# InternetMaximalism/plonky2_bn254

Hardware: AMD Instinct MI355X
Metric: G1 scalar-mul STARK proofs/sec (256-bit scalars) (higher is better)
Workload: dtype u64 (Goldilocks p = 2^64-2^32+1; BN254 Fq as 10x26-bit Montgomery limbs); 1 GPU; configs[1]: batch of 1024 G1 scalar-muls on 1 GPU per step = 8 proofs x 128 instances, 2^16 rows, W=781, standard_fast_config; instances_per_proof=128, steps_in_flight=4, parallelism=1 GPU, no collective

## Files before the change

plonky2_bn254_amd/csrc/quotient_common.h:

```cpp
#pragma once
#include "gl_dev.h"
#include "aux.h"

struct Acc {
  u64 lo, hi;
  u32 ov;
};
__device__ __forceinline__ void acc_init(Acc& a) {
  a.lo = 0;
  a.hi = 0;
  a.ov = 0;
}
__device__ __forceinline__ void acc_mad(Acc& a, u64 x, u64 w) {
  const unsigned __int128 pr = (unsigned __int128)x * w;
  u64 pl = (u64)pr, ph = (u64)(pr >> 64);
  a.lo += pl;
  u64 c = a.lo < pl ? 1 : 0;
  u64 h = a.hi + ph;
  u32 o = h < ph ? 1 : 0;
  h += c;
  o += h < c ? 1 : 0;
  a.hi = h;
  a.ov += o;
}
__device__ __forceinline__ u64 acc_red(const Acc& a) {
  return gl_sub(gl_reduce128(a.lo, a.hi), ((u64)a.ov) << 32);
}
struct Acc2 {
  Acc a0, a1;
};
__device__ __forceinline__ void acc2_init(Acc2& a) {
  acc_init(a.a0);
  acc_init(a.a1);
}
__device__ __forceinline__ void acc2_mad(Acc2& a, u64 x, u64 w0, u64 w1) {
  acc_mad(a.a0, x, w0);
  acc_mad(a.a1, x, w1);
}

static constexpr u32 M22 = (1u << 22) - 1;
struct W3 {
  u32 w0, w1, w2;
};
GL_HD W3 w3_split(u64 w) {
  W3 r;
  r.w0 = (u32)w & M22;
  r.w1 = (u32)(w >> 22) & M22;
  r.w2 = (u32)(w >> 44);
  return r;
}
struct Acc3 {
  u64 c[5];
};
__device__ __forceinline__ void acc3_init(Acc3& a) {
#pragma unroll
  for (int k = 0; k < 5; k++) a.c[k] = 0;
}
__device__ __forceinline__ void acc3_mad(Acc3& a, u32 v0, u32 v1, u32 v2, u32 w0, u32 w1, u32 w2) {
  a.c[0] += (u64)v0 * w0;
  a.c[1] += (u64)v0 * w1;
  a.c[1] += (u64)v1 * w0;
  a.c[2] += (u64)v0 * w2;
  a.c[2] += (u64)v1 * w1;
  a.c[2] += (u64)v2 * w0;
  a.c[3] += (u64)v1 * w2;
  a.c[3] += (u64)v2 * w1;
  a.c[4] += (u64)v2 * w2;
}
__device__ __forceinline__ u64 acc3_red(const Acc3& a) {
  unsigned __int128 t = (unsigned __int128)a.c[0] + ((unsigned __int128)a.c[1] << 22) + ((unsigned __int128)a.c[2] << 44);
  u64 r = gl_reduce128((u64)t, (u64)(t >> 64));
  r = gl_add(r, gl_mul_2exp<66>(gl_reduce128(a.c[3], 0)));
  r = gl_add(r, gl_mul_2exp<88>(gl_reduce128(a.c[4], 0)));
  return r;
}

struct AccW {
  Acc3 a0, a1;
};
__device__ __forceinline__ void accw_init(AccW& a) {
  acc3_init(a.a0);
  acc3_init(a.a1);
}
__device__ __forceinline__ void accw_mad(AccW& a, u64 x, const u32* __restrict__ w) {
  const u32 v0 = (u32)x & M22, v1 = (u32)(x >> 22) & M22, v2 = (u32)(x >> 44);
  acc3_mad(a.a0, v0, v1, v2, w[0], w[1], w[2]);
  acc3_mad(a.a1, v0, v1, v2, w[4], w[5], w[6]);
}
GL_HD void w3_store(u64* dst , u64 wa, u64 wb) {
  const W3 a = w3_split(wa), b = w3_split(wb);
  dst[0] = (u64)a.w0 | ((u64)a.w1 << 32);
  dst[1] = (u64)a.w2;
  dst[2] = (u64)b.w0 | ((u64)b.w1 << 32);
  dst[3] = (u64)b.w2;
}

struct QPointTables {
  const u64* x;
  const u64* lfirst;
  const u64* llast;
};

__device__ __forceinline__ size_t next_position(size_t j, unsigned log_n) {
  const size_t N = (size_t)1 << log_n;
  size_t h = j >> log_n;
  u32 k = bitrev32((u32)(j & (N - 1)), log_n);
  k = (k + 1) & (u32)(N - 1);
  return (h << log_n) | bitrev32(k, log_n);
}

__device__ __forceinline__ void lookup_and_ctl_constraints(const StarkShape& sh, const u64* __restrict__ tl,
                                                           const u64* __restrict__ al, size_t M2, size_t j, size_t jn,
                                                           const u32* __restrict__ W3 , int e0,
                                                           const u64 betas[2], const u64 gammas[2], u64 lfirst, u64 llast,
                                                           u64 z_last, u64& tot0, u64& tot1) {
  const int m = sh.n_helpers(), n_rc = sh.n_rc();
  int e = e0;
  AccW acc;
  accw_init(acc);
  const u64 table = tl[(size_t)sh.table_col * M2 + j], freq = tl[(size_t)sh.freq_col * M2 + j];
  u64 hs[2] = {0, 0};
#pragma unroll 4
  for (int k = 0; k < m; k++) {
    u64 f0 = tl[(size_t)(sh.rc_begin + 2 * k) * M2 + j];
    bool two = (2 * k + 1) < n_rc;
    u64 f1 = two ? tl[(size_t)(sh.rc_begin + 2 * k + 1) * M2 + j] : 0;
#pragma unroll
    for (int ch = 0; ch < 2; ch++) {
      u64 h = al[(size_t)(ch * (m + 1) + k) * M2 + j];
      u64 g0 = gl_add(f0, betas[ch]);
      u64 c;
      if (two) {
        u64 g1 = gl_add(f1, betas[ch]);
        c = gl_sub(gl_sub(gl_mul(gl_mul(g1, g0), h), g1), g0);
      } else {
        c = gl_sub(gl_mul(g0, h), 1);
      }
      int ee = e0 + ch * (m + 2) + k;
      accw_mad(acc, c, W3 + 8 * (ee));
      hs[ch] = gl_add(hs[ch], h);
    }
  }
#pragma unroll
  for (int ch = 0; ch < 2; ch++) {
    u64 z = al[(size_t)(ch * (m + 1) + m) * M2 + j], nz = al[(size_t)(ch * (m + 1) + m) * M2 + jn];
    u64 twc = gl_add(table, betas[ch]);
    u64 y = gl_sub(gl_mul(hs[ch], twc), freq);
    int ee = e0 + ch * (m + 2) + m;
    accw_mad(acc, gl_mul(z, lfirst), W3 + 8 * (ee));
    accw_mad(acc, gl_sub(gl_mul(gl_sub(nz, z), twc), y), W3 + 8 * (ee + 1));
  }
  e = e0 + 2 * (m + 2);
  for (int ctl = 0; ctl < sh.n_ctl; ctl++) {
    u64 a0 = 0, a1 = 0;
    for (int mm = sh.ctl.ncols[ctl] - 1; mm >= 0; mm--) {
      int start = sh.ctl.col_start[ctl][mm], nb = sh.ctl.col_bits[ctl][mm];
      u64 v = 0;
      for (int b = nb - 1; b >= 0; b--) v = gl_add(gl_dbl(v), tl[(size_t)(start + b) * M2 + j]);
      a0 = gl_add(gl_mul(a0, betas[0]), v);
      a1 = gl_add(gl_mul(a1, betas[1]), v);
    }
    u64 comb[2] = {gl_add(a0, gammas[0]), gl_add(a1, gammas[1])};
    u64 f0 = tl[(size_t)sh.ctl.filter_col[ctl] * M2 + j];
#pragma unroll
    for (int ch = 0; ch < 2; ch++) {
      int zc = 2 * (m + 1) + ctl * 2 + ch;
      u64 lz = al[(size_t)zc * M2 + j], nz = al[(size_t)zc * M2 + jn];
      u64 c_last = gl_mul(gl_sub(gl_mul(comb[ch], lz), f0), llast);
      u64 c_tr = gl_mul(gl_sub(gl_mul(comb[ch], gl_sub(lz, nz)), f0), z_last);
      accw_mad(acc, c_last, W3 + 8 * (e));
      accw_mad(acc, c_tr, W3 + 8 * (e + 1));
      e += 2;
    }
  }
  tot0 = gl_add(tot0, acc3_red(acc.a0));
  tot1 = gl_add(tot1, acc3_red(acc.a1));
}
```

plonky2_bn254_amd/csrc/quotient_g1.hip:

```cpp
#include "quotient_sched.h"
#include "trace_g1.h"
#include "quotient.h"

static constexpr int G1_K_AIR = 1111;
static constexpr int G1_MZ_E0[5] = {0, 50, 83, 132, 165};

__global__ __launch_bounds__(256, 2) void k_quotient_g1_sched(QArgs A) {
  const size_t j = (size_t)blockIdx.x * blockDim.x + threadIdx.x;
  if (j >= A.count) return;
  schedule_part<G1L, false>(A, j, q_next(A, j), 198, 5);
}

template <int part>
__global__ __launch_bounds__(256, 2) void k_quotient_g1_add(QArgs A) {
  const size_t M2 = A.stride;
  const size_t j = (size_t)blockIdx.x * blockDim.x + threadIdx.x;
  if (j >= A.count) return;
  const u64* __restrict__ tl = A.tl;
  const u64* __restrict__ W0 = A.W;
  const u64* __restrict__ W1 = A.W + A.K;
  const u32* __restrict__ W3 = (const u32*)(A.W + 2 * (size_t)A.K);
  u64 tot0 = 0, tot1 = 0;
  int e = 0;
  const int AUX = G1_COL_AUX;
  const u64 filter = TL(G1_COL_FILTER);
  const u64 is_x_eq_filter = TL(AUX + G1_AUX_IS_X_EQ_FILTER);
  u64 ax[16], lam[16], t16[16], u16[16];
  ld16(tl, M2, j, G1_COL_A, ax);
  if constexpr (part == 0) {
    const u64 is_x_eq = TL(AUX + G1_AUX_IS_X_EQ);
    ld16(tl, M2, j, G1_COL_B, u16);
#pragma unroll
    for (int i = 0; i < 16; i++) u16[i] = gl_sub(u16[i], ax[i]);
    ld16(tl, M2, j, AUX + G1_AUX_IS_X_EQ_AUX, t16);
    const u64 c0 = gl_sub(is_x_eq, 1);
    mz_block<true>(tl, M2, j, AUX + G1_AUX_IS_X_EQ_AUX + 16, A, G1_MZ_E0[0], 0,
             filter, [&](int i) __attribute__((always_inline)) { u64 v = conv16<true>(u16, t16, i); return i == 0 ? gl_add(v, c0) : v; }, tot0, tot1);
    e = 33;
    AccW g;
    accw_init(g);
#pragma unroll
    for (int i = 0; i < 16; i++) accw_mad(g, u16[i], W3 + 8 * (e + i));
    e += 16;
    u64 f = gl_mul(filter, is_x_eq);
    tot0 = gl_add(tot0, gl_mul(f, acc3_red(g.a0)));
    tot1 = gl_add(tot1, gl_mul(f, acc3_red(g.a1)));
    EMIT(gl_sub(gl_mul(filter, is_x_eq), is_x_eq_filter));
  } else if constexpr (part == 1) {
    ld16(tl, M2, j, AUX + G1_AUX_LAMBDA, lam);
    ld16(tl, M2, j, G1_COL_B, u16);
#pragma unroll
    for (int i = 0; i < 16; i++) u16[i] = gl_sub(u16[i], ax[i]);
    ld16(tl, M2, j, G1_COL_B + 16, t16);
    ld16(tl, M2, j, G1_COL_A + 16, ax);
    mz_block<true>(tl, M2, j, AUX + G1_AUX_LAMBDA_AUX, A, G1_MZ_E0[1], 1,
             gl_sub(filter, is_x_eq_filter),
             [&](int i) __attribute__((always_inline)) {
               u64 v = conv16<true>(lam, u16, i);
               return i < 16 ? gl_sub(v, gl_sub(t16[i < 16 ? i : 0], ax[i < 16 ? i : 0])) : v;
             },
             tot0, tot1);
  } else if constexpr (part == 2) {
    ld16(tl, M2, j, AUX + G1_AUX_LAMBDA, lam);
    ld16(tl, M2, j, G1_COL_A + 16, u16);
    mz_block<true>(tl, M2, j, AUX + G1_AUX_LAMBDA_AUX, A, G1_MZ_E0[2], 2,
             is_x_eq_filter,
             [&](int i) __attribute__((always_inline)) {
               u64 ly = conv16<true>(lam, u16, i), xx = conv16<true>(ax, ax, i);
               return gl_sub(gl_dbl(ly), gl_add(gl_dbl(xx), xx));
             },
             tot0, tot1);
    e = 116;
    ld16(tl, M2, j, G1_COL_B + 16, t16);
    AccW g;
    accw_init(g);
#pragma unroll
    for (int i = 0; i < 16; i++) accw_mad(g, gl_sub(u16[i], t16[i]), W3 + 8 * (e + i));
    tot0 = gl_add(tot0, gl_mul(is_x_eq_filter, acc3_red(g.a0)));
    tot1 = gl_add(tot1, gl_mul(is_x_eq_filter, acc3_red(g.a1)));
  } else if constexpr (part == 3) {
    ld16(tl, M2, j, AUX + G1_AUX_LAMBDA, lam);
    ld16(tl, M2, j, G1_COL_B, t16);
    ld16(tl, M2, j, G1_COL_C, u16);
    mz_block<true>(tl, M2, j, AUX + G1_AUX_X_AUX, A, G1_MZ_E0[3], 3, filter,
             [&](int i) __attribute__((always_inline)) {
               u64 v = conv16<true>(lam, lam, i);
               return i < 16 ? gl_sub(v, gl_add(gl_add(ax[i < 16 ? i : 0], t16[i < 16 ? i : 0]), u16[i < 16 ? i : 0])) : v;
             },
             tot0, tot1);
  } else {
    ld16(tl, M2, j, AUX + G1_AUX_LAMBDA, lam);
    ld16(tl, M2, j, G1_COL_C, u16);
#pragma unroll
    for (int i = 0; i < 16; i++) u16[i] = gl_sub(u16[i], ax[i]);
    ld16(tl, M2, j, G1_COL_C + 16, t16);
    ld16(tl, M2, j, G1_COL_A + 16, ax);
    mz_block<true>(tl, M2, j, AUX + G1_AUX_Y_AUX, A, G1_MZ_E0[4], 4, filter,
             [&](int i) __attribute__((always_inline)) {
               u64 v = conv16<true>(lam, u16, i);
               return i < 16 ? gl_add(v, gl_add(t16[i < 16 ? i : 0], ax[i < 16 ? i : 0])) : v;
             },
             tot0, tot1);
  }
  store_part(A, part, j, tot0, tot1);
}

__global__ __launch_bounds__(256) void k_quotient_finish(QArgs A, StarkShape sh) {
  const size_t j = (size_t)blockIdx.x * blockDim.x + threadIdx.x;
  if (j >= A.count) return;
  finish_point(A, sh, j);
}
void quotient_finish_launch(const QArgs& A, const StarkShape& sh, hipStream_t st) {
  k_quotient_finish<<<(unsigned)((A.count + 255) / 256), 256, 0, st>>>(A, sh);
}

__global__ void k_point_tables(u64* x, u64* lfirst, u64* llast, unsigned log_n, u64 w_n, u64 w_2n) {
  const size_t N = (size_t)1 << log_n;
  size_t j = (size_t)blockIdx.x * blockDim.x + threadIdx.x;
  if (j >= 2 * N) return;
  size_t h = j >> log_n;
  u32 k = bitrev32((u32)(j & (N - 1)), log_n);
  u64 shift = h ? gl_mul(GL_GEN, w_2n) : GL_GEN;
  u64 xv = gl_mul(shift, gl_pow(w_n, k));
  u64 gn = gl_pow(GL_GEN, N);
  u64 zh = gl_sub(h ? gl_neg(gn) : gn, 1);
  u64 ninv = gl_inv((u64)N % GL_P);
  u64 winv = gl_inv(w_n);
  x[j] = xv;
  lfirst[j] = gl_mul(gl_mul(zh, ninv), gl_inv(gl_sub(xv, 1)));
  llast[j] = gl_mul(gl_mul(gl_mul(zh, ninv), winv), gl_inv(gl_sub(xv, winv)));
}

__global__ void k_point_tables_window(u64* x, u64* lfirst, u64* llast, unsigned log_n, u32 h, size_t k0, size_t count, u64 w_n,
                                      u64 w_2n) {
  const size_t N = (size_t)1 << log_n;
  size_t j = (size_t)blockIdx.x * blockDim.x + threadIdx.x;
  if (j >= count) return;
  const u64 k = (k0 + j) & (N - 1);
  u64 shift = h ? gl_mul(GL_GEN, w_2n) : GL_GEN;
  u64 xv = gl_mul(shift, gl_pow(w_n, k));
  u64 gn = gl_pow(GL_GEN, N);
  u64 zh = gl_sub(h ? gl_neg(gn) : gn, 1);
  u64 ninv = gl_inv((u64)N % GL_P);
  u64 winv = gl_inv(w_n);
  x[j] = xv;
  lfirst[j] = gl_mul(gl_mul(zh, ninv), gl_inv(gl_sub(xv, 1)));
  llast[j] = gl_mul(gl_mul(gl_mul(zh, ninv), winv), gl_inv(gl_sub(xv, winv)));
}
void quotient_point_tables_window(u64* d_x, u64* d_lfirst, u64* d_llast, unsigned log_n, int h, size_t k0, size_t count, hipStream_t st) {
  k_point_tables_window<<<(unsigned)((count + 255) / 256), 256, 0, st>>>(d_x, d_lfirst, d_llast, log_n, (u32)h, k0, count,
                                                                       gl_root_of_unity(log_n), gl_root_of_unity(log_n + 1));
}
void quotient_window_args(QArgs& A, const u64* d_tw, const u64* d_aw, const QPointTables& pt, u64* d_part, size_t stride, size_t count,
                          size_t k0, int h) {
  A.tl = d_tw;
  A.al = d_aw;
  A.pt = pt;
  A.part = d_part;
  A.stride = stride;
  A.count = count;
  A.k0 = k0;
  A.natural = 1;
  A.hsel = (u32)h;
}

void quotient_point_tables(u64* d_x, u64* d_lfirst, u64* d_llast, unsigned log_n, hipStream_t st) {
  size_t M2 = (size_t)2 << log_n;
  k_point_tables<<<(unsigned)((M2 + 255) / 256), 256, 0, st>>>(d_x, d_lfirst, d_llast, log_n, gl_root_of_unity(log_n),
                                                             gl_root_of_unity(log_n + 1));
}

void quotient_host_tables(int K, const u64 alphas[2], const int* mz_e0, int n_blocks, std::vector<u64>& W, std::vector<u64>& mzt) {
  W.assign(QUOTIENT_W_WORDS(K), 0);
  for (int a = 0; a < 2; a++) {
    u64 v = 1;
    for (int e = K - 1; e >= 0; e--) {
      W[(size_t)a * K + e] = v;
      v = gl_mul(v, alphas[a]);
    }
  }
  static const u64 MOD[16] = {64839, 55420, 35862, 15392, 51853, 26737, 27281, 38785,
                              22621, 33153, 17846, 47184, 41001, 57649, 20082, 12388};
  const u64 B = 1ULL << 16, OFF = 1ULL << 29;
  mzt.assign(QUOTIENT_MZT_WORDS, 0);
  for (int blk = 0; blk < n_blocks; blk++)
    for (int a = 0; a < 2; a++) {
      const u64* w = &W[(size_t)a * K + mz_e0[blk] + 1];
      u64* T = &mzt[(size_t)(blk * 2 + a) * 80];
      for (int jj = 0; jj < 17; jj++) {
        u64 s = 0;
        for (int t = 0; t < 16; t++)
          if (jj + t < 32) s = gl_add(s, gl_mul(w[jj + t], MOD[t]));
        T[jj] = s;
      }
      u64 usum = 0;
      for (int d = 0; d < 31; d++) {
        u64 u = gl_sub(w[d + 1], gl_mul(B, w[d]));
        T[17 + d] = u;
        T[48 + d] = gl_mul(B, u);
        usum = gl_add(usum, u);
      }
      T[79] = gl_mul(OFF, usum);
    }
  for (int e = 0; e < K; e++) w3_store(&W[2 * (size_t)K + 4 * (size_t)e], W[e], W[(size_t)K + e]);
  for (int blk = 0; blk < n_blocks; blk++)
    for (int t = 0; t < 80; t++)
      w3_store(&mzt[QUOTIENT_MZT3_OFF + (size_t)(blk * 80 + t) * 4], mzt[(size_t)(blk * 2) * 80 + t], mzt[(size_t)(blk * 2 + 1) * 80 + t]);
}

void quotient_fill_args(QArgs& A, const StarkShape& sh, const u64* d_tl, const u64* d_al, const u64* d_W, const u64* d_mzt,
                        const QPointTables& pt, const u64 betas[2], const u64 gammas[2], unsigned log_n, u64* d_out,
                        u64* d_part) {
  A.tl = d_tl;
  A.al = d_al;
  A.W = d_W;
  A.mzt = d_mzt;
  A.pt = pt;
  for (int i = 0; i < 2; i++) {
    A.betas[i] = betas[i];
    A.gammas[i] = gammas[i];
  }
  const size_t N = (size_t)1 << log_n;
  u64 gn = gl_pow(GL_GEN, N);
  A.zh_inv[0] = gl_inv(gl_sub(gn, 1));
  A.zh_inv[1] = gl_inv(gl_sub(gl_neg(gn), 1));
  A.w_inv = gl_inv(gl_root_of_unity(log_n));
  A.out = d_out;
  A.part = d_part;
  A.n_parts = 0;
  A.log_n = log_n;
  A.K = sh.n_total_constraints();
  A.stride = A.count = 2 * N;
  A.k0 = 0;
  A.natural = 0;
  A.hsel = 0;
}

int g1_quotient_mz_blocks(const int** e0) {
  *e0 = G1_MZ_E0;
  return 5;
}
void g1_quotient_launch(const QArgs& A0, const StarkShape& sh, hipStream_t st) {
  QArgs A = A0;
  A.n_parts = 6;
  const unsigned g = (unsigned)((A.count + 255) / 256);
  k_quotient_g1_add<0><<<g, 256, 0, st>>>(A);
  k_quotient_g1_add<1><<<g, 256, 0, st>>>(A);
  k_quotient_g1_add<2><<<g, 256, 0, st>>>(A);
  k_quotient_g1_add<3><<<g, 256, 0, st>>>(A);
  k_quotient_g1_add<4><<<g, 256, 0, st>>>(A);
  k_quotient_g1_sched<<<g, 256, 0, st>>>(A);
  quotient_finish_launch(A, sh, st);
}

void quotient_g1_module_warm() {
  hipFuncAttributes a;
  (void)hipFuncGetAttributes(&a, reinterpret_cast<const void*>(&k_point_tables));
}
```

plonky2_bn254_amd/csrc/quotient_g2fq.hip:

```cpp
#include "quotient_sched.h"
#include "quotient.h"

static constexpr int G2_MZ_E0[10] = {1, 50, 100, 133, 166, 199, 264, 297, 330, 363};
static constexpr int FQ_MZ_E0[1] = {0};

__device__ __forceinline__ u64 econv_c0(const u64* x0, const u64* x1, const u64* y0, const u64* y1, int i) {
  return gl_sub(conv16(x0, y0, i), conv16(x1, y1, i));
}
__device__ __forceinline__ u64 econv_c1(const u64* x0, const u64* x1, const u64* y0, const u64* y1, int i) {
  return gl_add(conv16(x0, y1, i), conv16(x1, y0, i));
}

#define MZB(blk, auxcol, FILTER, FN, ...) \
  mz_block(tl, M2, j, (auxcol), A, G2_MZ_E0[blk], (blk), (FILTER), FN, tot0, tot1, ##__VA_ARGS__)

__global__ __launch_bounds__(256, 2) void k_quotient_g2_sched(QArgs A) {
  const size_t j = (size_t)blockIdx.x * blockDim.x + threadIdx.x;
  if (j >= A.count) return;
  schedule_part<G2L, false>(A, j, q_next(A, j), 396, 6);
}

template <int part>
__global__ __launch_bounds__(256, 2) void k_quotient_g2_add(QArgs A) {
  typedef G2L L;
  const size_t M2 = A.stride;
  const size_t j = (size_t)blockIdx.x * blockDim.x + threadIdx.x;
  if (j >= A.count) return;
  const u64* __restrict__ tl = A.tl;
  const u64* __restrict__ W0 = A.W;
  const u64* __restrict__ W1 = A.W + A.K;
  const u32* __restrict__ W3 = (const u32*)(A.W + 2 * (size_t)A.K);
  u64 tot0 = 0, tot1 = 0;
  int e = 0;
  const u64 filter = TL(L::FILTER);
  const int AUX = L::AUX;
  u64 is_x_eq_filter = 0;
  if constexpr (part == 1 || part == 2) is_x_eq_filter = TL(AUX + G2_AUX_IS_X_EQ_FILTER);
  auto seed_w = [&](Acc2& sd, int blk, int i, u64 v) { acc2_mad(sd, v, W0[G2_MZ_E0[blk] + 1 + i], W1[G2_MZ_E0[blk] + 1 + i]); };
  if constexpr (part == 0 || part == 5) {
    constexpr int h = part == 0 ? 0 : 1;
    u64 dx[16], t0[16];
    const u64 z = TL(AUX + (h ? G2_AUX_IS_C1_ZERO : G2_AUX_IS_C0_ZERO));
    if constexpr (h == 0) {
      EMIT(gl_mul(filter, gl_sub(gl_mul(z, TL(AUX + G2_AUX_IS_C1_ZERO)), TL(AUX + G2_AUX_IS_X_EQ))));
    }
#pragma unroll
    for (int i = 0; i < 16; i++) dx[i] = gl_sub(TL(L::B + 16 * h + i), TL(L::A + 16 * h + i));
    ld16(tl, M2, j, AUX + (h ? G2_AUX_C1_AUX : G2_AUX_C0_AUX), t0);
    const u64 c0 = gl_sub(z, 1);
    MZB(h, AUX + (h ? G2_AUX_C1_AUX : G2_AUX_C0_AUX) + 16, filter, [&](int i) __attribute__((always_inline)) { u64 v = conv16(dx, t0, i); return i == 0 ? gl_add(v, c0) : v; });
    e = h ? 83 : 34;
    AccW g;
    accw_init(g);
#pragma unroll
    for (int i = 0; i < 16; i++) accw_mad(g, dx[i], W3 + 8 * (e + i));
    const u64 f = gl_mul(filter, z);
    tot0 = gl_add(tot0, gl_mul(f, acc3_red(g.a0)));
    tot1 = gl_add(tot1, gl_mul(f, acc3_red(g.a1)));
    if constexpr (h == 1) {
      e = 99;
      EMIT(gl_sub(gl_mul(filter, TL(AUX + G2_AUX_IS_X_EQ)), TL(AUX + G2_AUX_IS_X_EQ_FILTER)));
    }
  } else {
    Acc2 sd0, sd1;
    acc2_init(sd0);
    acc2_init(sd1);
    u64 l0[16], l1[16], dx0[16], dx1[16];
    if constexpr (part == 1) {
#pragma unroll 4
      for (int i = 0; i < 16; i++) seed_w(sd0, 2, i, gl_sub(TL(L::A + 32 + i), TL(L::B + 32 + i)));
      ld16(tl, M2, j, AUX + G2_AUX_LAMBDA, l0);
      ld16(tl, M2, j, AUX + G2_AUX_LAMBDA + 16, l1);
#pragma unroll
      for (int i = 0; i < 16; i++) {
        dx0[i] = gl_sub(TL(L::B + i), TL(L::A + i));
        dx1[i] = gl_sub(TL(L::B + 16 + i), TL(L::A + 16 + i));
      }
      const u64 f_ne = gl_sub(filter, is_x_eq_filter);
      MZB(2, AUX + G2_AUX_LAMBDA_AUX, f_ne, [&](int i) __attribute__((always_inline)) { return econv_c0(l0, l1, dx0, dx1, i); }, &sd0);
#pragma unroll 4
      for (int i = 0; i < 16; i++) seed_w(sd1, 3, i, gl_sub(TL(L::A + 48 + i), TL(L::B + 48 + i)));
      MZB(3, AUX + G2_AUX_LAMBDA_AUX + 80, f_ne, [&](int i) __attribute__((always_inline)) { return econv_c1(l0, l1, dx0, dx1, i); }, &sd1);
    } else if constexpr (part == 2) {
      ld16(tl, M2, j, L::A, dx0);
      ld16(tl, M2, j, L::A + 16, dx1);
#pragma unroll
      for (int i = 0; i < 31; i++) {
        const u64 xx0 = econv_c0(dx0, dx1, dx0, dx1, i), xx1 = econv_c1(dx0, dx1, dx0, dx1, i);
        seed_w(sd0, 4, i, gl_neg(gl_add(gl_dbl(xx0), xx0)));
        seed_w(sd1, 5, i, gl_neg(gl_add(gl_dbl(xx1), xx1)));
      }
      ld16(tl, M2, j, AUX + G2_AUX_LAMBDA, l0);
      ld16(tl, M2, j, AUX + G2_AUX_LAMBDA + 16, l1);
      ld16(tl, M2, j, L::A + 32, dx0);
      ld16(tl, M2, j, L::A + 48, dx1);
      MZB(4, AUX + G2_AUX_LAMBDA_AUX, is_x_eq_filter, [&](int i) __attribute__((always_inline)) { return gl_dbl(econv_c0(l0, l1, dx0, dx1, i)); }, &sd0);
      MZB(5, AUX + G2_AUX_LAMBDA_AUX + 80, is_x_eq_filter, [&](int i) __attribute__((always_inline)) { return gl_dbl(econv_c1(l0, l1, dx0, dx1, i)); }, &sd1);
      e = 232;
      AccW g;
      accw_init(g);
#pragma unroll
      for (int i = 0; i < 16; i++) accw_mad(g, gl_sub(dx0[i], TL(L::B + 32 + i)), W3 + 8 * (e + i));
#pragma unroll
      for (int i = 0; i < 16; i++) accw_mad(g, gl_sub(dx1[i], TL(L::B + 48 + i)), W3 + 8 * (e + 16 + i));
      tot0 = gl_add(tot0, gl_mul(is_x_eq_filter, acc3_red(g.a0)));
      tot1 = gl_add(tot1, gl_mul(is_x_eq_filter, acc3_red(g.a1)));
    } else if constexpr (part == 3) {
#pragma unroll 4
      for (int i = 0; i < 16; i++) {
        seed_w(sd0, 6, i, gl_neg(gl_add(gl_add(TL(L::A + i), TL(L::B + i)), TL(L::C + i))));
        seed_w(sd1, 7, i, gl_neg(gl_add(gl_add(TL(L::A + 16 + i), TL(L::B + 16 + i)), TL(L::C + 16 + i))));
      }
      ld16(tl, M2, j, AUX + G2_AUX_LAMBDA, l0);
      ld16(tl, M2, j, AUX + G2_AUX_LAMBDA + 16, l1);
      MZB(6, AUX + G2_AUX_X_AUX, filter, [&](int i) __attribute__((always_inline)) { return econv_c0(l0, l1, l0, l1, i); }, &sd0);
      MZB(7, AUX + G2_AUX_X_AUX + 80, filter, [&](int i) __attribute__((always_inline)) { return econv_c1(l0, l1, l0, l1, i); }, &sd1);
    } else {
#pragma unroll 4
      for (int i = 0; i < 16; i++) seed_w(sd0, 8, i, gl_add(TL(L::C + 32 + i), TL(L::A + 32 + i)));
      ld16(tl, M2, j, AUX + G2_AUX_LAMBDA, l0);
      ld16(tl, M2, j, AUX + G2_AUX_LAMBDA + 16, l1);
#pragma unroll
      for (int i = 0; i < 16; i++) {
        dx0[i] = gl_sub(TL(L::C + i), TL(L::A + i));
        dx1[i] = gl_sub(TL(L::C + 16 + i), TL(L::A + 16 + i));
      }
      MZB(8, AUX + G2_AUX_Y_AUX, filter, [&](int i) __attribute__((always_inline)) { return econv_c0(l0, l1, dx0, dx1, i); }, &sd0);
#pragma unroll 4
      for (int i = 0; i < 16; i++) seed_w(sd1, 9, i, gl_add(TL(L::C + 48 + i), TL(L::A + 48 + i)));
      MZB(9, AUX + G2_AUX_Y_AUX + 80, filter, [&](int i) __attribute__((always_inline)) { return econv_c1(l0, l1, dx0, dx1, i); }, &sd1);
    }
  }
  store_part(A, part, j, tot0, tot1);
}

__global__ __launch_bounds__(256, 2) void k_quotient_fq_sched(QArgs A) {
  const size_t j = (size_t)blockIdx.x * blockDim.x + threadIdx.x;
  if (j >= A.count) return;
  schedule_part<FQL, true>(A, j, q_next(A, j), 33, 1);
}
__global__ __launch_bounds__(256) void k_quotient_fq_mul(QArgs A) {
  typedef FQL L;
  const size_t M2 = A.stride;
  const size_t j = (size_t)blockIdx.x * blockDim.x + threadIdx.x;
  if (j >= A.count) return;
  const u64* __restrict__ tl = A.tl;
  const u64* __restrict__ W0 = A.W;
  const u64* __restrict__ W1 = A.W + A.K;
  u64 tot0 = 0, tot1 = 0;
  const u64 filter = TL(L::FILTER);
  u64 a[16], b[16], c[16];
  ld16(tl, M2, j, L::A, a);
  ld16(tl, M2, j, L::B, b);
  ld16(tl, M2, j, L::C, c);
  mz_block(tl, M2, j, L::AUX, A, FQ_MZ_E0[0], 0, filter,
           [&](int i) __attribute__((always_inline)) {
             u64 v = conv16(a, b, i);
             return i < 16 ? gl_sub(v, c[i < 16 ? i : 0]) : v;
           },
           tot0, tot1);
  store_part(A, 0, j, tot0, tot1);
}

int g2_quotient_mz_blocks(const int** e0) {
  *e0 = G2_MZ_E0;
  return 10;
}
int fq_quotient_mz_blocks(const int** e0) {
  *e0 = FQ_MZ_E0;
  return 1;
}
void g2_quotient_launch(const QArgs& A0, const StarkShape& sh, hipStream_t st) {
  QArgs A = A0;
  A.n_parts = 7;
  const unsigned g = (unsigned)((A.count + 255) / 256);
  k_quotient_g2_add<0><<<g, 256, 0, st>>>(A);
  k_quotient_g2_add<5><<<g, 256, 0, st>>>(A);
  k_quotient_g2_add<1><<<g, 256, 0, st>>>(A);
  k_quotient_g2_add<2><<<g, 256, 0, st>>>(A);
  k_quotient_g2_add<3><<<g, 256, 0, st>>>(A);
  k_quotient_g2_add<4><<<g, 256, 0, st>>>(A);
  k_quotient_g2_sched<<<g, 256, 0, st>>>(A);
  quotient_finish_launch(A, sh, st);
}
void fq_quotient_launch(const QArgs& A0, const StarkShape& sh, hipStream_t st) {
  QArgs A = A0;
  A.n_parts = 2;
  const unsigned g = (unsigned)((A.count + 255) / 256);
  k_quotient_fq_mul<<<g, 256, 0, st>>>(A);
  k_quotient_fq_sched<<<g, 256, 0, st>>>(A);
  quotient_finish_launch(A, sh, st);
}

void quotient_g2fq_module_warm() {
  hipFuncAttributes a;
  (void)hipFuncGetAttributes(&a, reinterpret_cast<const void*>(&k_quotient_fq_sched));
}
```

plonky2_bn254_amd/csrc/quotient_sched.h:

```cpp
#pragma once
#include <vector>
#include "quotient_common.h"
#include "layout.h"

#ifndef MZ_CONSTS
#define MZ_CONSTS
static constexpr int QMZ_IQP = 0, QMZ_QUOT = 1, QMZ_LO = 18, QMZ_HI = 49;
#endif

struct QArgs {
  const u64* tl;
  const u64* al;
  const u64* W;
  const u64* mzt;
  QPointTables pt;
  u64 betas[2], gammas[2];
  u64 zh_inv[2];
  u64 w_inv;
  u64* out;
  u64* part;
  int n_parts;
  unsigned log_n;
  int K;
  size_t stride, count, k0;
  u32 natural, hsel;
};
static constexpr size_t QUOTIENT_MZT3_OFF = 10 * 2 * 80, QUOTIENT_MZT_WORDS = 10 * 2 * 80 + 10 * 80 * 4;
static inline size_t QUOTIENT_W_WORDS(int K) { return 6 * (size_t)K; }
__device__ __forceinline__ size_t q_next(const QArgs& A, size_t j) { return A.natural ? j + 1 : next_position(j, A.log_n); }

#define TL(c) tl[(size_t)(c)*M2 + j]
#define TN(c) tl[(size_t)(c)*M2 + jn]

__device__ __forceinline__ void ld16(const u64* __restrict__ tl, size_t M2, size_t j, int col, u64* v) {
#pragma unroll
  for (int i = 0; i < 16; i++) v[i] = tl[(size_t)(col + i) * M2 + j];
}
template <bool FULL = false>
__device__ __forceinline__ u64 conv16(const u64* A, const u64* B, int i) {
  Acc a;
  acc_init(a);
  if constexpr (FULL) {
#pragma clang loop unroll(full)
    for (int s = 0; s < 16; s++) {
      int t = i - s;
      if (t >= 0 && t < 16) acc_mad(a, A[s], B[t]);
    }
  } else {
#pragma unroll
    for (int s = 0; s < 16; s++) {
      int t = i - s;
      if (t >= 0 && t < 16) acc_mad(a, A[s], B[t]);
    }
  }
  return acc_red(a);
}

template <bool FULL = false, class InFn>
__device__ __forceinline__ void mz_block(const u64* __restrict__ tl, size_t M2, size_t j, int auxcol, const QArgs& A, int e0, int blk,
                                         u64 filter, InFn in, u64& tot0, u64& tot1, const Acc2* seed = nullptr) {
  const u64* __restrict__ w0 = A.W + e0;
  const u64* __restrict__ w1 = A.W + A.K + e0;
  const u64* __restrict__ T0 = A.mzt + (size_t)blk * 160;
  const u64* __restrict__ T1 = T0 + 80;
  const u32* __restrict__ w3 = (const u32*)(A.W + 2 * (size_t)A.K) + 8 * (size_t)e0;
  const u32* __restrict__ T3 = (const u32*)(A.mzt + QUOTIENT_MZT3_OFF) + 8 * (size_t)(blk * 80);
  u64 n0, n1;
  {
    Acc2 neg;
    if (seed) neg = *seed;
    else acc2_init(neg);
    if constexpr (FULL) {
#pragma clang loop unroll(full)
      for (int i = 0; i < 31; i++) acc2_mad(neg, in(i), w0[1 + i], w1[1 + i]);
    } else {
#pragma unroll
      for (int i = 0; i < 31; i++) {
        acc2_mad(neg, in(i), w0[1 + i], w1[1 + i]);
        __builtin_amdgcn_sched_barrier(0);
      }
    }
    n0 = acc_red(neg.a0);
    n1 = acc_red(neg.a1);
  }
  __builtin_amdgcn_sched_barrier(0);
  const u64 iqp = TL(auxcol + QMZ_IQP);
  const u64 qsign = gl_sub(gl_dbl(iqp), 1);
  u64 s0, s1;
  {
    AccW q;
    accw_init(q);
#pragma unroll 1
    for (int jj = 0; jj < 17; jj++) accw_mad(q, TL(auxcol + QMZ_QUOT + jj), T3 + 8 * jj);
    s0 = gl_mul(qsign, acc3_red(q.a0));
    s1 = gl_mul(qsign, acc3_red(q.a1));
  }
  __builtin_amdgcn_sched_barrier(0);
  {
    AccW pos;
    accw_init(pos);
    accw_mad(pos, gl_sub(gl_mul(iqp, iqp), iqp), w3);
#pragma unroll 1
    for (int d = 0; d < 31; d++) {
      accw_mad(pos, TL(auxcol + QMZ_LO + d), T3 + 8 * (17 + d));
      accw_mad(pos, TL(auxcol + QMZ_HI + d), T3 + 8 * (48 + d));
    }
    s0 = gl_add(s0, acc3_red(pos.a0));
    s1 = gl_add(s1, acc3_red(pos.a1));
  }
  s0 = gl_sub(gl_sub(s0, T0[79]), n0);
  s1 = gl_sub(gl_sub(s1, T1[79]), n1);
  tot0 = gl_add(tot0, gl_mul(filter, s0));
  tot1 = gl_add(tot1, gl_mul(filter, s1));
  asm volatile("" : "+v"(tot0), "+v"(tot1));
}

#define EQ_GROUP(filter, n, AEXPR, BEXPR)                         \
  {                                                               \
    static_assert((n) % 16 == 0, "EQ_GROUP: n % 16");             \
    AccW g_;                                                      \
    accw_init(g_);                                                \
    constexpr int CH_ = 16;                                       \
    _Pragma("unroll 1") for (int i0_ = 0; i0_ < (n); i0_ += CH_) { \
      u64 d_[CH_];                                                \
      _Pragma("unroll") for (int k_ = 0; k_ < CH_; k_++) {        \
        const int i = i0_ + k_;                                   \
        d_[k_] = gl_sub((AEXPR), (BEXPR));                        \
      }                                                           \
      _Pragma("unroll") for (int k_ = 0; k_ < CH_; k_++) accw_mad(g_, d_[k_], W3 + 8 * (e + i0_ + k_)); \
    }                                                             \
    e += (n);                                                     \
    u64 f_ = (filter);                                            \
    tot0 = gl_add(tot0, gl_mul(f_, acc3_red(g_.a0)));             \
    tot1 = gl_add(tot1, gl_mul(f_, acc3_red(g_.a1)));             \
    asm volatile("" : "+v"(tot0), "+v"(tot1));  \
  }
#define EMIT(c)                                  \
  {                                              \
    u64 c_ = (c);                                \
    tot0 = gl_add(tot0, gl_mul(c_, W0[e]));      \
    tot1 = gl_add(tot1, gl_mul(c_, W1[e]));      \
    e += 1;                                      \
  }


__device__ __forceinline__ void store_part(const QArgs& A, int part, size_t j, u64 tot0, u64 tot1) {
  const size_t M2 = A.stride;
  A.part[((size_t)part * 2 + 0) * M2 + j] = tot0;
  A.part[((size_t)part * 2 + 1) * M2 + j] = tot1;
}

template <class L, bool FIRST_A_IS_ONE>
__device__ __forceinline__ void schedule_part(const QArgs& A, size_t j, size_t jn, int e, int part) {
  u64 tot0 = 0, tot1 = 0;
  const size_t M2 = A.stride;
  const u64* __restrict__ tl = A.tl;
  const u64* __restrict__ W0 = A.W;
  const u64* __restrict__ W1 = A.W + A.K;
  const u32* __restrict__ W3 = (const u32*)(A.W + 2 * (size_t)A.K);
  const u64 filter = TL(L::FILTER);
  const u64 is_first = TL(L::FLAGS + 0), is_last = TL(L::FLAGS + 1);
  const u64 n_filter = TN(L::FILTER), n_is_last = TN(L::FLAGS + 1);
  const u64 is_not_last_round = gl_sub(filter, is_last);
  const u64 is_next_not_last_round = gl_sub(n_filter, n_is_last);
  const u64 is_adding = TL(L::IS_ADDING), idnl = TL(L::IDNL);
  const u64 n_is_adding = TN(L::IS_ADDING), n_idnl = TN(L::IDNL);
  const u64 bit0 = TL(L::BITS), n_bit0 = TN(L::BITS);

  EMIT(gl_mul(is_first, gl_sub(is_adding, 1)));
  EQ_GROUP(is_first, L::PL, TL(L::DOUBLE + i), TL(L::B + i));
  EQ_GROUP(gl_mul(bit0, is_first), L::PL, TL(L::SUM + i), TL(L::C + i));
  EQ_GROUP(gl_mul(gl_sub(1, bit0), is_first), L::PL, TL(L::SUM + i), TL(L::A + i));
  if (FIRST_A_IS_ONE) {
    EQ_GROUP(is_first, L::PL, TL(L::A + i), (u64)(i == 0 ? 1 : 0));
  }
  EQ_GROUP(idnl, L::PL, TN(L::A + i), TL(L::SUM + i));
  EQ_GROUP(idnl, L::PL, TN(L::B + i), TL(L::DOUBLE + i));
  EQ_GROUP(gl_mul(n_bit0, idnl), L::PL, TN(L::SUM + i), TN(L::C + i));
  EQ_GROUP(gl_mul(gl_sub(1, n_bit0), idnl), L::PL, TN(L::SUM + i), TN(L::A + i));
  EQ_GROUP(idnl, L::PL, TN(L::DOUBLE + i), TL(L::DOUBLE + i));
  EMIT(gl_mul(idnl, gl_sub(n_is_adding, 1)));
  EMIT(gl_mul(idnl, n_idnl));
  EQ_GROUP(idnl, 256, TN(L::BITS + i), TL(L::BITS + ((i + 1) & 255)));
  EQ_GROUP(is_adding, L::PL, TN(L::A + i), TL(L::DOUBLE + i));
  EQ_GROUP(is_adding, L::PL, TN(L::B + i), TL(L::DOUBLE + i));
  EQ_GROUP(is_adding, L::PL, TN(L::SUM + i), TL(L::SUM + i));
  EQ_GROUP(is_adding, L::PL, TN(L::DOUBLE + i), TN(L::C + i));
  EMIT(gl_mul(is_adding, n_is_adding));
  EMIT(gl_mul(is_adding, gl_sub(n_idnl, is_next_not_last_round)));
  EQ_GROUP(is_adding, 256, TN(L::BITS + i), TL(L::BITS + i));
  {
    const u64 counter = TL(L::FLAGS + 2), inv_c = TL(L::FLAGS + 3), inv_cp = TL(L::FLAGS + 4);
    const u64 n_counter = TN(L::FLAGS + 2);
    const u64 not_filter = gl_sub(1, filter);
    EMIT(gl_mul(not_filter, is_first));
    EMIT(gl_mul(not_filter, is_last));
    EMIT(gl_mul(filter, gl_sub(gl_mul(counter, inv_c), gl_sub(1, is_first))));
    EMIT(gl_mul(gl_mul(filter, counter), is_first));
    const u64 cp = gl_sub(counter, 511);
    EMIT(gl_mul(filter, gl_sub(gl_mul(cp, inv_cp), gl_sub(1, is_last))));
    EMIT(gl_mul(gl_mul(filter, cp), is_last));
    EMIT(gl_mul(gl_mul(filter, gl_sub(1, is_last)), gl_sub(gl_sub(n_counter, counter), 1)));
    EMIT(gl_mul(gl_mul(filter, is_last), n_counter));
  }
  EMIT(gl_mul(is_not_last_round, gl_sub(TN(L::TIMESTAMP), TL(L::TIMESTAMP))));
  EMIT(gl_mul(is_not_last_round, gl_sub(n_filter, filter)));
  const u64 x = A.pt.x[j], llast = A.pt.llast[j];
  const u64 z_last = gl_sub(x, A.w_inv);
  {
    const u64 rc = TL(L::RANGE), diff = gl_sub(TN(L::RANGE), rc);
    EMIT(gl_mul(gl_sub(gl_mul(diff, diff), diff), z_last));
    EMIT(gl_mul(gl_sub(rc, 65535), llast));
  }
  store_part(A, part, j, tot0, tot1);
}

__device__ __forceinline__ void finish_point(const QArgs& A, const StarkShape& sh, size_t j) {
  const unsigned log_n = A.log_n;
  const size_t N = (size_t)1 << log_n, M2 = A.stride;
  const size_t jn = q_next(A, j);
  u64 tot0 = 0, tot1 = 0;
  for (int p = 0; p < A.n_parts; p++) {
    tot0 = gl_add(tot0, A.part[((size_t)p * 2 + 0) * M2 + j]);
    tot1 = gl_add(tot1, A.part[((size_t)p * 2 + 1) * M2 + j]);
  }
  const u64 x = A.pt.x[j], lfirst = A.pt.lfirst[j], llast = A.pt.llast[j];
  const u64 z_last = gl_sub(x, A.w_inv);
  lookup_and_ctl_constraints(sh, A.tl, A.al, M2, j, jn, (const u32*)(A.W + 2 * (size_t)A.K), sh.n_constraints, A.betas, A.gammas,
                             lfirst, llast, z_last, tot0, tot1);
  const size_t h = A.natural ? A.hsel : j >> log_n;
  const size_t k = A.natural ? A.k0 + j : (size_t)bitrev32((u32)(j & (N - 1)), log_n);
  A.out[(0 * 2 + h) * N + k] = gl_mul(tot0, A.zh_inv[h]);
  A.out[(1 * 2 + h) * N + k] = gl_mul(tot1, A.zh_inv[h]);
}

void quotient_host_tables(int K, const u64 alphas[2], const int* mz_e0, int n_blocks, std::vector<u64>& W, std::vector<u64>& mzt);
void quotient_fill_args(QArgs& A, const StarkShape& sh, const u64* d_tl, const u64* d_al, const u64* d_W, const u64* d_mzt,
                        const QPointTables& pt, const u64 betas[2], const u64 gammas[2], unsigned log_n, u64* d_out,
                        u64* d_part);
static constexpr int QUOTIENT_MAX_PARTS = 7;
void quotient_finish_launch(const QArgs& A, const StarkShape& sh, hipStream_t st);
```

Baseline: 86.41 proofs/s.

## Fuse G1 quotient part kernels into one 2D launch and use constant address space

Replaces six separate G1 quotient kernel launches with one launch whose blockIdx.y selects the part. This cuts launch overhead and lets the parts run concurrently on the GPU. Weight and table pointers are cast to address space 4 (constant), so the compiler can use scalar loads for these uniform values. Per-element subtractions are hoisted out of the convolution lambdas, and register barriers are added in the unrolled accumulation loop. The barriers constrain scheduling and may change register pressure.

```diff
diff --git a/plonky2_bn254_amd/csrc/quotient_common.h b/plonky2_bn254_amd/csrc/quotient_common.h
--- a/plonky2_bn254_amd/csrc/quotient_common.h
+++ b/plonky2_bn254_amd/csrc/quotient_common.h
@@ -82,7 +82,8 @@
   acc3_init(a.a0);
   acc3_init(a.a1);
 }
-__device__ __forceinline__ void accw_mad(AccW& a, u64 x, const u32* __restrict__ w) {
+template <class WP>
+__device__ __forceinline__ void accw_mad(AccW& a, u64 x, WP w) {
   const u32 v0 = (u32)x & M22, v1 = (u32)(x >> 22) & M22, v2 = (u32)(x >> 44);
   acc3_mad(a.a0, v0, v1, v2, w[0], w[1], w[2]);
   acc3_mad(a.a1, v0, v1, v2, w[4], w[5], w[6]);
diff --git a/plonky2_bn254_amd/csrc/quotient_g1.hip b/plonky2_bn254_amd/csrc/quotient_g1.hip
--- a/plonky2_bn254_amd/csrc/quotient_g1.hip
+++ b/plonky2_bn254_amd/csrc/quotient_g1.hip
@@ -5,21 +5,13 @@
 static constexpr int G1_K_AIR = 1111;
 static constexpr int G1_MZ_E0[5] = {0, 50, 83, 132, 165};
 
-__global__ __launch_bounds__(256, 2) void k_quotient_g1_sched(QArgs A) {
-  const size_t j = (size_t)blockIdx.x * blockDim.x + threadIdx.x;
-  if (j >= A.count) return;
-  schedule_part<G1L, false>(A, j, q_next(A, j), 198, 5);
-}
-
 template <int part>
-__global__ __launch_bounds__(256, 2) void k_quotient_g1_add(QArgs A) {
+__device__ __forceinline__ void g1_add_part(const QArgs& A, size_t j) {
   const size_t M2 = A.stride;
-  const size_t j = (size_t)blockIdx.x * blockDim.x + threadIdx.x;
-  if (j >= A.count) return;
   const u64* __restrict__ tl = A.tl;
-  const u64* __restrict__ W0 = A.W;
-  const u64* __restrict__ W1 = A.W + A.K;
-  const u32* __restrict__ W3 = (const u32*)(A.W + 2 * (size_t)A.K);
+  const qc64 W0 = QCONST(u64, A.W);
+  const qc64 W1 = QCONST(u64, A.W + A.K);
+  const qc32 W3 = QCONST(u32, A.W + 2 * (size_t)A.K);
   u64 tot0 = 0, tot1 = 0;
   int e = 0;
   const int AUX = G1_COL_AUX;
@@ -53,11 +45,13 @@
     for (int i = 0; i < 16; i++) u16[i] = gl_sub(u16[i], ax[i]);
     ld16(tl, M2, j, G1_COL_B + 16, t16);
     ld16(tl, M2, j, G1_COL_A + 16, ax);
+#pragma unroll
+    for (int i = 0; i < 16; i++) t16[i] = gl_sub(t16[i], ax[i]);
     mz_block<true>(tl, M2, j, AUX + G1_AUX_LAMBDA_AUX, A, G1_MZ_E0[1], 1,
              gl_sub(filter, is_x_eq_filter),
              [&](int i) __attribute__((always_inline)) {
                u64 v = conv16<true>(lam, u16, i);
-               return i < 16 ? gl_sub(v, gl_sub(t16[i < 16 ? i : 0], ax[i < 16 ? i : 0])) : v;
+               return i < 16 ? gl_sub(v, t16[i < 16 ? i : 0]) : v;
              },
              tot0, tot1);
   } else if constexpr (part == 2) {
@@ -82,10 +76,12 @@
     ld16(tl, M2, j, AUX + G1_AUX_LAMBDA, lam);
     ld16(tl, M2, j, G1_COL_B, t16);
     ld16(tl, M2, j, G1_COL_C, u16);
+#pragma unroll
+    for (int i = 0; i < 16; i++) ax[i] = gl_add(gl_add(ax[i], t16[i]), u16[i]);
     mz_block<true>(tl, M2, j, AUX + G1_AUX_X_AUX, A, G1_MZ_E0[3], 3, filter,
              [&](int i) __attribute__((always_inline)) {
                u64 v = conv16<true>(lam, lam, i);
-               return i < 16 ? gl_sub(v, gl_add(gl_add(ax[i < 16 ? i : 0], t16[i < 16 ? i : 0]), u16[i < 16 ? i : 0])) : v;
+               return i < 16 ? gl_sub(v, ax[i < 16 ? i : 0]) : v;
              },
              tot0, tot1);
   } else {
@@ -95,14 +91,29 @@
     for (int i = 0; i < 16; i++) u16[i] = gl_sub(u16[i], ax[i]);
     ld16(tl, M2, j, G1_COL_C + 16, t16);
     ld16(tl, M2, j, G1_COL_A + 16, ax);
+#pragma unroll
+    for (int i = 0; i < 16; i++) t16[i] = gl_add(t16[i], ax[i]);
     mz_block<true>(tl, M2, j, AUX + G1_AUX_Y_AUX, A, G1_MZ_E0[4], 4, filter,
              [&](int i) __attribute__((always_inline)) {
                u64 v = conv16<true>(lam, u16, i);
-               return i < 16 ? gl_add(v, gl_add(t16[i < 16 ? i : 0], ax[i < 16 ? i : 0])) : v;
+               return i < 16 ? gl_add(v, t16[i < 16 ? i : 0]) : v;
              },
              tot0, tot1);
   }
   store_part(A, part, j, tot0, tot1);
+}
+
+__global__ __launch_bounds__(256, 2) void k_quotient_g1_parts(QArgs A) {
+  const size_t j = (size_t)blockIdx.x * blockDim.x + threadIdx.x;
+  if (j >= A.count) return;
+  switch (blockIdx.y) {
+    case 0: schedule_part<G1L, false>(A, j, q_next(A, j), 198, 5); break;
+    case 1: g1_add_part<0>(A, j); break;
+    case 2: g1_add_part<1>(A, j); break;
+    case 3: g1_add_part<2>(A, j); break;
+    case 4: g1_add_part<3>(A, j); break;
+    default: g1_add_part<4>(A, j); break;
+  }
 }
 
 __global__ __launch_bounds__(256) void k_quotient_finish(QArgs A, StarkShape sh) {
@@ -244,12 +255,7 @@
   QArgs A = A0;
   A.n_parts = 6;
   const unsigned g = (unsigned)((A.count + 255) / 256);
-  k_quotient_g1_add<0><<<g, 256, 0, st>>>(A);
-  k_quotient_g1_add<1><<<g, 256, 0, st>>>(A);
-  k_quotient_g1_add<2><<<g, 256, 0, st>>>(A);
-  k_quotient_g1_add<3><<<g, 256, 0, st>>>(A);
-  k_quotient_g1_add<4><<<g, 256, 0, st>>>(A);
-  k_quotient_g1_sched<<<g, 256, 0, st>>>(A);
+  k_quotient_g1_parts<<<dim3(g, 6), 256, 0, st>>>(A);
   quotient_finish_launch(A, sh, st);
 }
 
diff --git a/plonky2_bn254_amd/csrc/quotient_g2fq.hip b/plonky2_bn254_amd/csrc/quotient_g2fq.hip
--- a/plonky2_bn254_amd/csrc/quotient_g2fq.hip
+++ b/plonky2_bn254_amd/csrc/quotient_g2fq.hip
@@ -27,9 +27,9 @@
   const size_t j = (size_t)blockIdx.x * blockDim.x + threadIdx.x;
   if (j >= A.count) return;
   const u64* __restrict__ tl = A.tl;
-  const u64* __restrict__ W0 = A.W;
-  const u64* __restrict__ W1 = A.W + A.K;
-  const u32* __restrict__ W3 = (const u32*)(A.W + 2 * (size_t)A.K);
+  const qc64 W0 = QCONST(u64, A.W);
+  const qc64 W1 = QCONST(u64, A.W + A.K);
+  const qc32 W3 = QCONST(u32, A.W + 2 * (size_t)A.K);
   u64 tot0 = 0, tot1 = 0;
   int e = 0;
   const u64 filter = TL(L::FILTER);
@@ -145,8 +145,8 @@
   const size_t j = (size_t)blockIdx.x * blockDim.x + threadIdx.x;
   if (j >= A.count) return;
   const u64* __restrict__ tl = A.tl;
-  const u64* __restrict__ W0 = A.W;
-  const u64* __restrict__ W1 = A.W + A.K;
+  const qc64 W0 = QCONST(u64, A.W);
+  const qc64 W1 = QCONST(u64, A.W + A.K);
   u64 tot0 = 0, tot1 = 0;
   const u64 filter = TL(L::FILTER);
   u64 a[16], b[16], c[16];
diff --git a/plonky2_bn254_amd/csrc/quotient_sched.h b/plonky2_bn254_amd/csrc/quotient_sched.h
--- a/plonky2_bn254_amd/csrc/quotient_sched.h
+++ b/plonky2_bn254_amd/csrc/quotient_sched.h
@@ -29,6 +29,10 @@
 static inline size_t QUOTIENT_W_WORDS(int K) { return 6 * (size_t)K; }
 __device__ __forceinline__ size_t q_next(const QArgs& A, size_t j) { return A.natural ? j + 1 : next_position(j, A.log_n); }
 
+#define QCONST(T, p) ((const __attribute__((address_space(4))) T*)(p))
+typedef const __attribute__((address_space(4))) u64* qc64;
+typedef const __attribute__((address_space(4))) u32* qc32;
+
 #define TL(c) tl[(size_t)(c)*M2 + j]
 #define TN(c) tl[(size_t)(c)*M2 + jn]
 
@@ -59,12 +63,12 @@
 template <bool FULL = false, class InFn>
 __device__ __forceinline__ void mz_block(const u64* __restrict__ tl, size_t M2, size_t j, int auxcol, const QArgs& A, int e0, int blk,
                                          u64 filter, InFn in, u64& tot0, u64& tot1, const Acc2* seed = nullptr) {
-  const u64* __restrict__ w0 = A.W + e0;
-  const u64* __restrict__ w1 = A.W + A.K + e0;
-  const u64* __restrict__ T0 = A.mzt + (size_t)blk * 160;
-  const u64* __restrict__ T1 = T0 + 80;
-  const u32* __restrict__ w3 = (const u32*)(A.W + 2 * (size_t)A.K) + 8 * (size_t)e0;
-  const u32* __restrict__ T3 = (const u32*)(A.mzt + QUOTIENT_MZT3_OFF) + 8 * (size_t)(blk * 80);
+  const qc64 w0 = QCONST(u64, A.W + e0);
+  const qc64 w1 = QCONST(u64, A.W + A.K + e0);
+  const qc64 T0 = QCONST(u64, A.mzt + (size_t)blk * 160);
+  const qc64 T1 = T0 + 80;
+  const qc32 w3 = QCONST(u32, A.W + 2 * (size_t)A.K) + 8 * (size_t)e0;
+  const qc32 T3 = QCONST(u32, A.mzt + QUOTIENT_MZT3_OFF) + 8 * (size_t)(blk * 80);
   u64 n0, n1;
   {
     Acc2 neg;
@@ -72,7 +76,13 @@
     else acc2_init(neg);
     if constexpr (FULL) {
 #pragma clang loop unroll(full)
-      for (int i = 0; i < 31; i++) acc2_mad(neg, in(i), w0[1 + i], w1[1 + i]);
+      for (int i = 0; i < 31; i++) {
+        acc2_mad(neg, in(i), w0[1 + i], w1[1 + i]);
+        if (i % 8 == 7) {
+          asm volatile("" : "+v"(neg.a0.lo), "+v"(neg.a0.hi), "+v"(neg.a0.ov), "+v"(neg.a1.lo), "+v"(neg.a1.hi), "+v"(neg.a1.ov));
+          __builtin_amdgcn_sched_barrier(0);
+        }
+      }
     } else {
 #pragma unroll
       for (int i = 0; i < 31; i++) {
@@ -82,6 +92,7 @@
     }
     n0 = acc_red(neg.a0);
     n1 = acc_red(neg.a1);
+    asm volatile("" : "+v"(n0), "+v"(n1));
   }
   __builtin_amdgcn_sched_barrier(0);
   const u64 iqp = TL(auxcol + QMZ_IQP);
@@ -155,9 +166,9 @@
   u64 tot0 = 0, tot1 = 0;
   const size_t M2 = A.stride;
   const u64* __restrict__ tl = A.tl;
-  const u64* __restrict__ W0 = A.W;
-  const u64* __restrict__ W1 = A.W + A.K;
-  const u32* __restrict__ W3 = (const u32*)(A.W + 2 * (size_t)A.K);
+  const qc64 W0 = QCONST(u64, A.W);
+  const qc64 W1 = QCONST(u64, A.W + A.K);
+  const qc32 W3 = QCONST(u32, A.W + 2 * (size_t)A.K);
   const u64 filter = TL(L::FILTER);
   const u64 is_first = TL(L::FLAGS + 0), is_last = TL(L::FLAGS + 1);
   const u64 n_filter = TN(L::FILTER), n_is_last = TN(L::FLAGS + 1);
```

After: 89.73 proofs/s (median of 6 runs). 3.9% higher.
